# torognes/vsearch

Hardware: NVIDIA H100
Metric: usearch_global_gcups (higher is better)
Workload: dtype int16

## Files before the change

### include/vsg.h

```cpp
#ifndef VSG_H
#define VSG_H

#include <stddef.h>
#include <stdint.h>

#ifdef __cplusplus
extern "C" {
#endif

#define VSG_OK 0
#define VSG_ENODEVICE (-1)
#define VSG_ECUDA (-2)
#define VSG_EINVAL (-3)
#define VSG_ENOMEM (-4)
#define VSG_ECAP (-5)

#define VSG_SCORE_SENTINEL 32767

typedef struct vsg_ctx vsg_ctx;
typedef struct vsg_seqset vsg_seqset;
typedef struct vsg_index vsg_index;

typedef struct vsg_scoring {
  int64_t v[14];
// ... 15 lines not shown
int vsg_seqset_create(vsg_ctx * ctx, const char * cat, const int64_t * off, const int32_t * len,
                      int64_t n, int host, vsg_seqset ** out);
void vsg_seqset_destroy(vsg_seqset * s);
int64_t vsg_seqset_count(const vsg_seqset * s);
int vsg_seqset_dust(vsg_ctx * ctx, vsg_seqset * s);
int vsg_seqset_symbols(vsg_ctx * ctx, const vsg_seqset * s, uint8_t * out, int64_t cap);
int vsg_seqset_revcomp(vsg_ctx * ctx, const vsg_seqset * src, int64_t q0, int64_t n, vsg_seqset ** out);

int vsg_align_pairs(vsg_ctx * ctx, const vsg_seqset * queries, const vsg_seqset * targets,
                    int64_t npairs, const uint32_t * qidx, const uint32_t * tidx,
                    int16_t * score, uint16_t * aligned, uint16_t * matches,
                    uint16_t * mismatches, uint16_t * gaps, int32_t * trims,
                    char * cigar_buf, int64_t cigar_cap, int64_t * cigar_off);

int vsg_align_pairs_gated(vsg_ctx * ctx, const vsg_seqset * queries, const vsg_seqset * targets,
                          int64_t npairs, const uint32_t * qidx, const uint32_t * tidx,
                          int16_t * score, uint16_t * aligned, uint16_t * matches,
                          uint16_t * mismatches, uint16_t * gaps, int32_t * trims,
                          const int32_t * leader_of, double threshold, int iddef, int64_t * ck_counts);

#define VSG_STAT_SCORE 0
#define VSG_STAT_ALIGNED 1
#define VSG_STAT_MATCHES 2
#define VSG_STAT_MISMATCHES 3
#define VSG_STAT_GAPS 4
#define VSG_STAT_TRIM_LEFT 5
#define VSG_STAT_TRIM_RIGHT 6
#define VSG_STAT_CIGARLEN 7
#define VSG_STAT_WORDS 8

typedef struct vsg_profile {
  int64_t cells;
  int64_t fast_pairs;
  int64_t exact_pairs;
  int64_t fwd_launches;
  float fwd_ms;
  float traceback_ms;
  float rank_ms;
  float reserved;
  int64_t tb_skipped;
  int64_t tb_redone;
} vsg_profile;
int vsg_profile_reset(vsg_ctx * ctx);
int vsg_profile_get(vsg_ctx * ctx, vsg_profile * out);
int vsg_measure_int_peak(vsg_ctx * ctx, double * packed_lane_ops_per_s);

int vsg_index_create(vsg_ctx * ctx, const vsg_seqset * db, int wordlength, int mask_lower,
                     vsg_index ** out);
void vsg_index_destroy(vsg_index * ix);

int vsg_rank(vsg_ctx * ctx, const vsg_index * ix, const vsg_seqset * queries, int64_t q0,
             int64_t nq, int minwordmatches, int tophits, int mask_lower,
             uint32_t * cand_seqno, uint32_t * cand_count, int32_t * ncand);

typedef struct vsg_search_opts {
  double id;
  double weak_id;
  int32_t maxaccepts;
  int32_t maxrejects;
  int32_t wordlength;
  int32_t minwordmatches;
  int32_t iddef;
  int32_t strand_both;
  int32_t mask_lower;
  int32_t lazy;
  double minqt, maxqt;
  double minsl, maxsl;
  double maxid;
  double mid;
  double query_cov;
  double target_cov;
  int64_t maxsubs;
  int64_t maxgaps;
  int64_t mincols;
  int64_t maxdiffs;
  int32_t leftjust;
  int32_t rightjust;
  int64_t maxqsize;
  int64_t mintsize;
  double minsizeratio;
  double maxsizeratio;
  int32_t idprefix;
  int32_t idsuffix;
  int32_t self;
  int32_t selfid;
  int32_t qmask_dust;
  int32_t unoise;
  const int64_t * query_sizes;
  const int64_t * target_sizes;
  const int64_t * query_labels;
  const int64_t * target_labels;
  double unoise_alpha;
  int32_t sizeorder;
  int32_t reserved1;
} vsg_search_opts;

typedef struct vsg_search_result {
  int32_t target;
  int32_t matches;
  int32_t mismatches;
  int32_t gaps;
  int32_t alignment_length;
  int32_t query_length;
  int32_t target_length;
  int32_t accepted;
  int32_t strand;
// ... 324 lines not shown
```

### vsearch_b200/csrc/rank.cu

```cuda
#include "vsg_internal.h"
#include "rank_steps.cuh"

#include <cub/cub.cuh>
#include <thrust/iterator/transform_iterator.h>

#include <algorithm>
#include <cstdlib>
#include <cstring>
#include <mutex>

namespace vsg {

constexpr int CAND_CAP = 2048;
constexpr int TOPHITS_MAX = RANK_TOPHITS_MAX;
constexpr int SCAN_SEG_WORDS = 512;

template <bool FILL>
__global__ void index_build_kernel(DevSeqs db, int t0, int nt, int k, int mask_lower, int split,
                                   uint32_t * __restrict__ count ,
                                   const uint32_t * __restrict__ start, uint16_t * __restrict__ post)
{
  extern __shared__ uint32_t bitmap[];
  int const lt = blockIdx.x;
  if (lt >= nt) { return; }
  int const words = (1 << (2 * k)) >> 5;
  for (int i = threadIdx.x; i < (words > 0 ? words : 1); i += blockDim.x) { bitmap[i] = 0; }
  __syncthreads();
  int64_t const t = static_cast<int64_t>(t0) + lt;
  const uint8_t * __restrict__ s = db.sym + db.off[t];
  int const len = db.len[t];
  for (int p = k - 1 + threadIdx.x; p < len; p += blockDim.x) {
    uint32_t km;
    if (kmer_at(s, p, k, mask_lower, km)) {
      uint32_t const bit = 1u << (km & 31);
      uint32_t const old = atomicOr(&bitmap[km >> 5], bit);
      if ((old & bit) == 0) {
        uint32_t const list = split ? 2u * km + static_cast<uint32_t>(lt & 1) : km;
        if (FILL) {
          uint32_t const pos = atomicAdd(&count[list], 1u);
          post[static_cast<size_t>(start[list]) + pos] = static_cast<uint16_t>((lt & ~1) << 1);
        } else {
          atomicAdd(&count[list], 1u);
        }
      }
    }
  }
}

__global__ void pad_counts_kernel(uint32_t * __restrict__ count, int n)
{
  int const i = blockIdx.x * blockDim.x + threadIdx.x;
  if (i < n) { count[i] = (count[i] + 7u) & ~7u; }
}
__global__ void fill_u16_kernel(uint16_t * __restrict__ p, size_t n, uint16_t v)
{
  size_t const i = static_cast<size_t>(blockIdx.x) * blockDim.x + threadIdx.x;
  if (i < n) { p[i] = v; }
}

__global__ void add_totals_kernel(const uint32_t * __restrict__ count , uint32_t * __restrict__ totals, size_t hashsize)
{
  size_t const i = static_cast<size_t>(blockIdx.x) * blockDim.x + threadIdx.x;
  if (i < hashsize) { totals[i] += count[2 * i] + count[2 * i + 1]; }
}

__global__ void shard_word_counts_kernel(ShardDev S, uint32_t nlists, uint32_t * __restrict__ totals)
{
  uint32_t const i = blockIdx.x * blockDim.x + threadIdx.x;
// ... 74 lines not shown
      else { int const v2 = vr - rem * (full + 1); lane = rem + v2 / full; blk = v2 % full; }
      lp[8 * (blk * 32 + lane) + j] = x;
    }
    __syncthreads();
  }
}

template <typename T, bool DESC>
__device__ void bitonic_sort_shared(T * a, int n )
{
  for (int size = 2; size <= n; size <<= 1) {
    for (int stride = size >> 1; stride > 0; stride >>= 1) {
      __syncthreads();
      for (int i = threadIdx.x; i < (n >> 1); i += blockDim.x) {
        int const lo = 2 * i - (i & (stride - 1));
        int const hi = lo + stride;
        bool const up = ((lo & size) == 0);
        T const x = a[lo], y = a[hi];
        bool const sw = DESC ? (up ? (x < y) : (x > y)) : (up ? (x > y) : (x < y));
        if (sw) { a[lo] = y; a[hi] = x; }
      }
    }
  }
  __syncthreads();
}

__device__ __forceinline__ int next_pow2(int v)
{
  int p = 1;
  while (p < v) { p <<= 1; }
  return p;
}


__device__ __forceinline__ int threshold_from_hist(const uint32_t * hist, int top, int floor, int tophits, int & K)
{
  int const lane = threadIdx.x & 31;
  int acc = 0;
  for (; top >= floor; top -= 32) {
    int const b = top - lane;
    int const v = warp_inclusive_sum(b >= floor ? static_cast<int>(hist[b]) : 0);
    unsigned const hit = __ballot_sync(0xffffffffu, acc + v >= tophits);
    if (hit != 0u) {
      int const first = __ffs(hit) - 1;
      K = acc + __shfl_sync(0xffffffffu, v, first);
      return top - first;
    }
    acc += __shfl_sync(0xffffffffu, v, 31);
  }
  K = acc;
  return floor;
}

__device__ __forceinline__ int keep_keys_from(uint64_t * cand, int m, uint64_t tkey, int & s_ncand)
{
  uint64_t mine[CAND_CAP / RANK_THREADS];
  int cnt = 0;
  for (int i = threadIdx.x; i < m; i += blockDim.x) { uint64_t const kx = cand[i]; if (kx >= tkey) { mine[cnt++] = kx; } }
  if (threadIdx.x == 0) { s_ncand = 0; }
  __syncthreads();
  int const base = cnt > 0 ? atomicAdd(&s_ncand, cnt) : 0;
  for (int i = 0; i < cnt; i++) { cand[base + i] = mine[i]; }
  __syncthreads();
  return s_ncand;
}

__device__ __forceinline__ int sort_and_cut(uint64_t * cand, int m, int tophits)
{
  int const p2 = next_pow2(m);
  for (int i = m + threadIdx.x; i < p2; i += blockDim.x) { cand[i] = 0; }
  bitonic_sort_shared<uint64_t, true>(cand, p2);
  return m < tophits ? m : tophits;
}


__device__ __forceinline__ int query_kmers_smem(const uint8_t * __restrict__ s, int nwin, int k, int mask_lower,
                                                uint32_t * kmers, uint32_t * flag, int & s_nk, int & np2)
{
  np2 = next_pow2(nwin > 1 ? nwin : 1);
  for (int i = threadIdx.x; i < np2; i += blockDim.x) {
    uint32_t km = 0xffffffffu;
    if (i < nwin) {
      uint32_t v;
      if (kmer_at(s, i + k - 1, k, mask_lower, v)) { km = v; }
    }
    kmers[i] = km;
  }
  bitonic_sort_shared<uint32_t, false>(kmers, np2);
  int mine = 0;
  for (int i = threadIdx.x; i < np2; i += blockDim.x) {
    uint32_t const v = kmers[i];
    bool const keep = (v != 0xffffffffu) && (i == 0 || kmers[i - 1] != v);
    flag[i] = keep ? 1u : 0u;
    mine += keep;
  }
  __syncthreads();
  for (int i = threadIdx.x; i < np2; i += blockDim.x) { if (flag[i] == 0u) { kmers[i] = 0xffffffffu; } }
  atomicAdd(&s_nk, mine);
  __syncthreads();
  return s_nk;
}

__device__ __forceinline__ int query_kmers_hbm(const uint8_t * __restrict__ s, int nwin, int k, int mask_lower,
                                               uint32_t * bm, int words, uint32_t * gk, int & s_nk)
{
  if (k <= 10) {
    for (int i = threadIdx.x; i < words; i += blockDim.x) { bm[i] = 0; }
    __syncthreads();
    for (int p = threadIdx.x; p < nwin; p += blockDim.x) {
      uint32_t v;
      if (kmer_at(s, p + k - 1, k, mask_lower, v)) {
        uint32_t const bit = 1u << (v & 31);
        uint32_t const old = atomicOr(&bm[v >> 5], bit);
        if ((old & bit) == 0) { gk[atomicAdd(&s_nk, 1)] = v; }
      }
    }
  } else {
    uint32_t const hmask = static_cast<uint32_t>(words) - 1u;
    for (int i = threadIdx.x; i < words; i += blockDim.x) { bm[i] = 0xffffffffu; }
    __syncthreads();
    for (int p = threadIdx.x; p < nwin; p += blockDim.x) {
      uint32_t v;
      if (kmer_at(s, p + k - 1, k, mask_lower, v)) {
        uint32_t slot = (v * 2654435761u) >> 7 & hmask;
        for (;;) {
          uint32_t const old = atomicCAS(&bm[slot], 0xffffffffu, v);
          if (old == 0xffffffffu) { gk[atomicAdd(&s_nk, 1)] = v; break; }
          if (old == v) { break; }
          slot = (slot + 1u) & hmask;
        }
      }
    }
  }
  __threadfence_block();
  __syncthreads();
  return s_nk;
}

__device__ __forceinline__ void postings_incr(const ShardDev & S, int n, const uint32_t * lbeg, const uint32_t * llen,
                                              uint32_t * counters)
{
  int const lane = threadIdx.x & 31, warp = threadIdx.x >> 5;
  for (int li = warp; li < n; li += RANK_THREADS / 32) {
    uint32_t const len = llen[li];
    const uint32_t * __restrict__ pl = S.post32 + lbeg[li];
    for (uint32_t e = lane; e < len; e += 32) {
      uint32_t const a = __ldg(pl + e) - static_cast<uint32_t>(S.t0);
      atomicAdd(&counters[a >> 1], (a & 1) ? 0x10000u : 1u);
    }
  }
}

enum { RANK_TOP = 0, RANK_COUNT = 1, RANK_EMIT = 2 };

template <bool INCR, int MODE = RANK_TOP>
__global__ void __launch_bounds__(RANK_THREADS, 2)
rank_kernel(DevSeqs qs, int64_t q0, int nq, DevSeqs db, const ShardDev * __restrict__ shards, int nshards,
            int k, int mask_lower, int minwordmatches, int tophits,
            uint32_t * __restrict__ out_seqno, uint32_t * __restrict__ out_count, int32_t * __restrict__ out_n,
            int32_t * __restrict__ status, uint32_t * __restrict__ scratch, size_t scratch_stride, int bitmap_words,
            const int64_t * __restrict__ key_off, uint64_t * __restrict__ keys)
{
  extern __shared__ __align__(16) unsigned char smem[];
  uint64_t * const cand = reinterpret_cast<uint64_t *>(smem);
  uint32_t * const counters = reinterpret_cast<uint32_t *>(smem + CAND_CAP * 8);
  uint32_t * const kmers = counters + COUNTER_WORDS + 3;
  uint32_t * const lbeg = kmers + KMER_CAP;
  uint32_t * const llen = lbeg + KMER_CAP;
  uint32_t * const cum = llen + KMER_CAP;
  __shared__ int s_ncand, s_nk, s_T, s_K;
  __shared__ int s_wsum[RANK_THREADS / 32];

  int const lane = threadIdx.x & 31, warp = threadIdx.x >> 5;

  bool clean = false;
  for (int qi = blockIdx.x; qi < nq; qi += gridDim.x) {
    int64_t const q = q0 + qi;
    const uint8_t * __restrict__ s = qs.sym + qs.off[q];
    int const len = qs.len[q];
    int const nwin = len - k + 1;
    if (threadIdx.x == 0) { s_ncand = 0; s_nk = 0; }
    bool const longq = nwin > KMER_CAP;
    if (longq && (scratch == nullptr || nwin > 65535)) {
      if (threadIdx.x == 0) { out_n[qi] = 0; atomicExch(status, 1); }
      continue;
    }
    int np2, nk, nchunks = 1;
    uint32_t * gk = nullptr;
    if (!longq) {
      nk = query_kmers_smem(s, nwin, k, mask_lower, kmers, lbeg, s_nk, np2);
    } else {
      uint32_t * const bm = scratch + static_cast<size_t>(blockIdx.x) * scratch_stride;
      gk = bm + bitmap_words;
      nk = query_kmers_hbm(s, nwin, k, mask_lower, bm, bitmap_words, gk, s_nk);
      nchunks = nk > 0 ? (nk + KMER_CAP - 1) / KMER_CAP : 1;
      np2 = 1;
    }
    uint32_t const minmatches = static_cast<uint32_t>(minwordmatches < nk ? minwordmatches : nk);
    bool const running = MODE == RANK_TOP && !longq && (np2 + nk + 1 <= KMER_CAP);
    uint32_t * const hist = kmers + np2;
    if (running) {
      for (int i = threadIdx.x; i <= nk; i += blockDim.x) { hist[i] = 0; }
      if (threadIdx.x == 0) { s_T = static_cast<int>(minmatches); }
    }

    for (int sh = 0; sh < nshards; sh++) {
      ShardDev const S = shards[sh];
      if (!clean) { for (int i = threadIdx.x; i < COUNTER_WORDS; i += blockDim.x) { counters[i] = 0; } }
      clean = false;
      for (int chunk = 0; chunk < nchunks; chunk++) {
        if (longq) {
          int const cn = nk > 0 ? min(KMER_CAP, nk - chunk * KMER_CAP) : 1;
          for (int i = threadIdx.x; i < cn; i += blockDim.x) { kmers[i] = nk > 0 ? gk[chunk * KMER_CAP + i] : 0xffffffffu; }
          np2 = cn;
          __syncthreads();
        }
        list_bounds<INCR>(S, kmers, np2, lbeg, llen);
        __syncthreads();
        if constexpr (INCR) { postings_incr(S, np2, lbeg, llen, counters); }
        else { postings_stream(S, np2, lbeg, llen, cum, counters, s_wsum); }
        __syncthreads();
      }
      int const nwords = (S.nt + 1) >> 1;
      uint32_t thr = minmatches;
      if constexpr (MODE != RANK_TOP) {
        visit_counters<4>(counters, 0, nwords, S.nt, minmatches, true, [&](uint32_t c, int lt) {
          int const pos = atomicAdd(&s_ncand, 1);
          if (MODE == RANK_EMIT) { keys[key_off[qi] + pos] = target_key(db, S, c, lt); }
        });
        clean = true;
        __syncthreads();
        continue;
      }
      if (running) {
        uint32_t const T0 = static_cast<uint32_t>(s_T);
        visit_counters<4>(counters, 0, nwords, S.nt, T0, false, [&](uint32_t c, int) { atomicAdd(&hist[c], 1u); });
        __syncthreads();
        if (warp == 0) {
          int K;
          int const T = threshold_from_hist(hist, nk, static_cast<int>(T0), tophits, K);
          if (lane == 0) { s_T = T; s_K = K; }
        }
        int const level = s_ncand;
        __syncthreads();
        uint32_t const T1 = static_cast<uint32_t>(s_T);
        if (level + s_K <= CAND_CAP) {
          visit_counters<4>(counters, 0, nwords, S.nt, T1, true, [&](uint32_t c, int lt) {
            cand[atomicAdd(&s_ncand, 1)] = target_key(db, S, c, lt);
          });
          clean = true;
          __syncthreads();
          continue;
        }
        thr = T1;
      } else {
        int mine = 0;
        visit_counters<1>(counters, 0, nwords, S.nt, minmatches, false, [&](uint32_t, int) { mine++; });
        int total;
        int pos = block_exclusive_sum(mine, s_wsum, total);
        int const level = s_ncand;
        __syncthreads();
        if (level + total <= CAND_CAP) {
          pos += level;
          visit_counters<1>(counters, 0, nwords, S.nt, minmatches, false, [&](uint32_t c, int lt) {
            cand[pos++] = target_key(db, S, c, lt);
          });
          if (threadIdx.x == 0) { s_ncand = level + total; }
          __syncthreads();
          continue;
        }
      }
      for (int seg = 0; seg < nwords; seg += SCAN_SEG_WORDS) {
        int const level = s_ncand;
        __syncthreads();
        if (level + 2 * SCAN_SEG_WORDS > CAND_CAP) {
          int const nkeep = sort_and_cut(cand, level, tophits);
          if (threadIdx.x == 0) { s_ncand = nkeep; }
          __syncthreads();
        }
        visit_counters<1>(counters, seg, min(seg + SCAN_SEG_WORDS, nwords), S.nt, thr, false, [&](uint32_t c, int lt) {
          cand[atomicAdd(&s_ncand, 1)] = target_key(db, S, c, lt);
        });
        __syncthreads();
      }
    }
    if constexpr (MODE != RANK_TOP) {
      if (threadIdx.x == 0) { out_n[qi] = s_ncand; }
      __syncthreads();
      continue;
    }
    int m = s_ncand;
    __syncthreads();
    if (m > 2 * tophits && nk + 1 <= 2 * KMER_CAP) {
      if (!running) {
        uint32_t * const hist5 = lbeg;
        for (int i = threadIdx.x; i <= nk; i += blockDim.x) { hist5[i] = 0; }
        __syncthreads();
        for (int i = threadIdx.x; i < m; i += blockDim.x) { atomicAdd(&hist5[static_cast<uint32_t>(cand[i] >> 49)], 1u); }
        __syncthreads();
        if (warp == 0) {
          int K;
          int const T = threshold_from_hist(hist5, nk, 0, tophits, K);
          if (lane == 0) { s_T = T; }
        }
        __syncthreads();
      }
      m = keep_keys_from(cand, m, count_key(s_T), s_ncand);
    }
    int const nout = sort_and_cut(cand, m, tophits);
    for (int i = threadIdx.x; i < nout; i += blockDim.x) {
      uint64_t const key = cand[i];
      out_seqno[static_cast<size_t>(qi) * tophits + i] = 0xffffffu - static_cast<uint32_t>(key & 0xffffffu);
      out_count[static_cast<size_t>(qi) * tophits + i] = static_cast<uint32_t>(key >> 49);
    }
    if (threadIdx.x == 0) { out_n[qi] = nout; }
    __syncthreads();
  }
}

constexpr size_t RANK_SMEM = CAND_CAP * 8 + (COUNTER_WORDS + 3) * 4 + KMER_CAP * 4 * 4 + 4;

}

using namespace vsg;

struct vsg_index {
  int device = 0;
  int k = 8;
  int mask_lower = 0;
  int64_t ntargets = 0;
  const vsg_seqset * db = nullptr;
  std::vector<DevBuf> b_start, b_post, b_rkeys;
  std::vector<ShardDev> h_shards;
  DevBuf b_shards;
  int64_t total_postings = 0;
  mutable std::mutex words_lock;
  mutable DevBuf b_words;
  mutable bool words_ready = false;
};

extern "C" void vsg_index_destroy(vsg_index * ix);
namespace vsg {

static void shard_bank_order(vsg_ctx * c, const uint32_t * start, uint16_t * post, size_t nlists)
{
  if (nlists == 0) { return; }
  int sms = 132;
  cudaDeviceGetAttribute(&sms, cudaDevAttrMultiProcessorCount, c->device);
  list_bank_order_kernel<<<static_cast<int>(std::min<size_t>(nlists, static_cast<size_t>(sms) * 32)), 128, 0, c->stream>>>(start, post, static_cast<int>(nlists));
  count_launch();
}

static int build_dense_shard(vsg_ctx * c, vsg_index * ix, int sh, int t0, int nt, DevBuf & cnt, DevBuf & tmp, uint32_t * d_totals)
{
  const vsg_seqset * db = ix->db;
  int const k = ix->k;
  size_t const hashsize = static_cast<size_t>(1) << (2 * k);
  size_t const bitmap_bytes = std::max<size_t>(hashsize / 8, 4);
  size_t const nlists = 2 * hashsize;
  int rc;
  int64_t nuc = 0;
  for (int i = 0; i < nt; i++) { nuc += db->h_len[static_cast<size_t>(t0) + static_cast<size_t>(i)]; }
  if (nuc + 7 * static_cast<int64_t>(nlists) >= (static_cast<int64_t>(1) << 32) - 64) {
    Error::set("vsg_index_create: a shard of 32766 targets holds 2^32 nucleotides or more");
    return VSG_EINVAL;
  }
  DevBuf & bs = ix->b_start[static_cast<size_t>(sh)];
  if ((rc = bs.reserve(sizeof(uint32_t) * (nlists + 1))) != VSG_OK) { return rc; }
  VSG_CUDA_OK(cudaMemsetAsync(cnt.p, 0, sizeof(uint32_t) * (nlists + 1), c->stream));
  index_build_kernel<false><<<nt, 128, bitmap_bytes, c->stream>>>(db->d, t0, nt, k, ix->mask_lower, 1,
                                                                  static_cast<uint32_t *>(cnt.p), nullptr, nullptr);
  count_launch();
  if (d_totals != nullptr) {
// ... 222 lines not shown
      count_launch();
    }
    VSG_CUDA_OK(cudaStreamSynchronize(c->stream));
    VSG_CUDA_OK(cudaGetLastError());
    ix->words_ready = true;
  }
  *out = static_cast<const uint32_t *>(ix->b_words.p);
  return VSG_OK;
}
const ShardDev * index_shards(const vsg_index * ix, int & nshards)
{
  nshards = static_cast<int>(ix->h_shards.size());
  return static_cast<const ShardDev *>(ix->b_shards.p);
}

static void rank_collect_time(vsg_ctx * c)
{
  if (c->rank_pending) {
    float ms = 0.f;
    if (cudaEventElapsedTime(&ms, c->ev[4], c->ev[5]) == cudaSuccess) { c->prof_rank_ms += ms; }
    c->rank_pending = false;
  }
}

static int rank_top_alloc(vsg_ctx * c, int64_t nq, int tophits, RankTop & r)
{
  size_t const cells = static_cast<size_t>(nq) * tophits;
  int rc;
  if ((rc = c->rank_tmp.reserve(sizeof(uint32_t) * (2 * cells + nq + 4))) != VSG_OK) { return rc; }
  r.seqno = static_cast<uint32_t *>(c->rank_tmp.p);
  r.count = r.seqno + cells;
  r.n = reinterpret_cast<int32_t *>(r.count + cells);
  r.status = r.n + nq;
  VSG_CUDA_OK(cudaMemsetAsync(r.status, 0, sizeof(int32_t), c->stream));
  return VSG_OK;
}

static int rank_status(int32_t status, const char * caller)
{
  if (status == 0) { return VSG_OK; }
  Error::set(std::string(caller) + ": a query is longer than the device ranker supports (65 534 + wordlength nt)");
  return VSG_EINVAL;
}

RankTargets index_targets(const vsg_index * ix, int mask_lower)
{
  RankTargets t;
  t.shards = static_cast<const ShardDev *>(ix->b_shards.p); t.nshards = static_cast<int>(ix->h_shards.size());
  t.lens = ix->db->d; t.k = ix->k; t.mask_lower = mask_lower; t.device = ix->device;
  t.incr = false; t.timed = true;
  return t;
}

template <int MODE>
static int rank_launch(vsg_ctx * c, const RankTargets & t, const vsg_seqset * queries, int64_t q0, int64_t nq,
                       int minwordmatches, int tophits, const RankTop & out, const int64_t * d_key_off, uint64_t * d_keys)
{
  int rc;
  auto const kernel = t.incr ? rank_kernel<true, MODE> : rank_kernel<false, MODE>;
  int const k = t.k;
  VSG_CUDA_OK(cudaFuncSetAttribute(kernel, cudaFuncAttributeMaxDynamicSharedMemorySize, static_cast<int>(RANK_SMEM)));
  int sms = 132;
  cudaDeviceGetAttribute(&sms, cudaDevAttrMultiProcessorCount, c->device);
  int const grid = static_cast<int>(std::min<int64_t>(nq, static_cast<int64_t>(sms) * 2));
  int maxlen = 0;
  for (int64_t q = q0; q < q0 + nq; q++) { maxlen = std::max(maxlen, queries->h_len[static_cast<size_t>(q)]); }
  uint32_t * d_scratch = nullptr;
  size_t stride = 0;
  int bitmap_words = std::max(1, (1 << (2 * std::min(k, 10))) >> 5);
  if (k > 10) { bitmap_words = 4096; while (bitmap_words < 2 * maxlen) { bitmap_words <<= 1; } }
  if (maxlen - k + 1 > KMER_CAP) {
    stride = static_cast<size_t>(bitmap_words) + static_cast<size_t>(maxlen) + 8;
    if ((rc = c->rank_scratch.reserve(sizeof(uint32_t) * stride * static_cast<size_t>(grid))) != VSG_OK) { return rc; }
    d_scratch = static_cast<uint32_t *>(c->rank_scratch.p);
  }
  if (t.timed) { VSG_CUDA_OK(cudaEventRecord(c->ev[4], c->stream)); }
  kernel<<<grid, RANK_THREADS, RANK_SMEM, c->stream>>>(
      queries->d, q0, static_cast<int>(nq), t.lens, t.shards, t.nshards, k, t.mask_lower, minwordmatches, tophits,
      out.seqno, out.count, out.n, out.status, d_scratch, stride, bitmap_words, d_key_off, d_keys);
  count_launch();
  if (t.timed) {
    VSG_CUDA_OK(cudaEventRecord(c->ev[5], c->stream));
    c->rank_pending = true;
  }
  return VSG_OK;
}

int rank_enqueue(vsg_ctx * c, const vsg_index * ix, const vsg_seqset * queries, int64_t q0, int64_t nq,
                 int minwordmatches, int tophits, int mask_lower, RankTop & out)
{
  if (tophits < 1 || tophits > TOPHITS_MAX) { Error::set("vsg_rank: tophits must be in 1..1024"); return VSG_EINVAL; }
  if (q0 < 0 || nq < 0 || q0 + nq > queries->d.n) { Error::set("vsg_rank: query range out of bounds"); return VSG_EINVAL; }
  if (queries->device != c->device || ix->device != c->device) { Error::set("vsg_rank: sequence set / index lives on another device than the context"); return VSG_EINVAL; }
  if (nq > (1 << 30) / tophits) { Error::set("vsg_rank: batch too large"); return VSG_EINVAL; }
  int rc;
  if ((rc = rank_top_alloc(c, nq, tophits, out)) != VSG_OK || nq == 0) { return rc; }
  return rank_launch<RANK_TOP>(c, index_targets(ix, mask_lower), queries, q0, nq, minwordmatches, tophits, out, nullptr, nullptr);
}

int rank_download(vsg_ctx * c, const RankTop & r, int64_t nq, int tophits, uint32_t * h_seqno, uint32_t * h_count,
                  int32_t * h_n, const char * caller)
{
  size_t const cells = static_cast<size_t>(nq) * tophits;
  int32_t status = 0;
  if (nq > 0) {
    VSG_CUDA_OK(cudaMemcpyAsync(h_seqno, r.seqno, sizeof(uint32_t) * cells, cudaMemcpyDeviceToHost, c->stream));
    VSG_CUDA_OK(cudaMemcpyAsync(h_count, r.count, sizeof(uint32_t) * cells, cudaMemcpyDeviceToHost, c->stream));
    VSG_CUDA_OK(cudaMemcpyAsync(h_n, r.n, sizeof(int32_t) * static_cast<size_t>(nq), cudaMemcpyDeviceToHost, c->stream));
  }
  VSG_CUDA_OK(cudaMemcpyAsync(&status, r.status, sizeof(int32_t), cudaMemcpyDeviceToHost, c->stream));
  VSG_CUDA_OK(cudaStreamSynchronize(c->stream));
  rank_collect_time(c);
  return rank_status(status, caller);
}

__global__ void cut_lists_kernel(const uint64_t * __restrict__ keys, const int64_t * __restrict__ key_off,
                                 const int64_t * __restrict__ out_off, uint32_t * __restrict__ seqno, uint32_t * __restrict__ count)
{
  int const q = blockIdx.x;
  int64_t const a = key_off[q], n = out_off[q + 1] - out_off[q], o = out_off[q];
  for (int64_t i = threadIdx.x; i < n; i += blockDim.x) {
    uint64_t const key = keys[a + i];
    seqno[o + i] = 0xffffffu - static_cast<uint32_t>(key & 0xffffffu);
    count[o + i] = static_cast<uint32_t>(key >> 49);
  }
}

int rank_counts(vsg_ctx * c, const RankTargets & t, const vsg_seqset * queries, int64_t q0, int64_t nq, int minwordmatches,
                std::vector<int32_t> & n)
{
// ... 60 lines not shown
      cub::DeviceSegmentedSort::SortKeysDescending(nullptr, tb, db, static_cast<int>(keys), static_cast<int>(m), d_koff, d_koff + 1, c->stream);
      if ((rc = c->cub_tmp.reserve(tb + 64)) != VSG_OK) { return rc; }
      cub::DeviceSegmentedSort::SortKeysDescending(c->cub_tmp.p, tb, db, static_cast<int>(keys), static_cast<int>(m), d_koff, d_koff + 1, c->stream);
      count_launch();
      if (nout > 0) {
        cut_lists_kernel<<<static_cast<unsigned>(m), 256, 0, c->stream>>>(db.Current(), d_koff, d_ooff, d_seq, d_cnt);
        count_launch();
        if (t.timed) { VSG_CUDA_OK(cudaEventRecord(c->ev[5], c->stream)); }
        size_t const o = static_cast<size_t>(first[static_cast<size_t>(a)]);
        VSG_CUDA_OK(cudaMemcpyAsync(seqno.data() + o, d_seq, sizeof(uint32_t) * static_cast<size_t>(nout), cudaMemcpyDeviceToHost, c->stream));
        VSG_CUDA_OK(cudaMemcpyAsync(count.data() + o, d_cnt, sizeof(uint32_t) * static_cast<size_t>(nout), cudaMemcpyDeviceToHost, c->stream));
      }
      VSG_CUDA_OK(cudaStreamSynchronize(c->stream));
      VSG_CUDA_OK(cudaGetLastError());
      rank_collect_time(c);
    }
    a = b;
  }
  return VSG_OK;
}

}

extern "C" int vsg_rank(vsg_ctx * c, const vsg_index * ix, const vsg_seqset * queries, int64_t q0, int64_t nq,
                        int minwordmatches, int tophits, int mask_lower, uint32_t * cand_seqno,
                        uint32_t * cand_count, int32_t * ncand)
{
  if (c == nullptr || ix == nullptr || queries == nullptr || cand_seqno == nullptr || cand_count == nullptr || ncand == nullptr) {
    Error::set("vsg_rank: null argument");
    return VSG_EINVAL;
  }
  VSG_CUDA_OK(cudaSetDevice(c->device));
  if (tophits > TOPHITS_MAX) {
    std::vector<int64_t> first;
    std::vector<uint32_t> seqno, count;
    int const rc = rank_lists(c, index_targets(ix, mask_lower), queries, q0, nq, minwordmatches, tophits, first, seqno, count);
    if (rc != VSG_OK) { return rc; }
    for (int64_t i = 0; i < nq; i++) {
      size_t const a = static_cast<size_t>(first[static_cast<size_t>(i)]), n = static_cast<size_t>(first[static_cast<size_t>(i) + 1]) - a;
      std::memcpy(cand_seqno + static_cast<size_t>(i) * tophits, seqno.data() + a, sizeof(uint32_t) * n);
      std::memcpy(cand_count + static_cast<size_t>(i) * tophits, count.data() + a, sizeof(uint32_t) * n);
      ncand[i] = static_cast<int32_t>(n);
    }
    return VSG_OK;
  }
  RankTop r;
  int rc = rank_enqueue(c, ix, queries, q0, nq, minwordmatches, tophits, mask_lower, r);
  if (rc == VSG_OK) { rc = rank_download(c, r, nq, tophits, cand_seqno, cand_count, ncand, "vsg_rank"); }
  if (rc != VSG_OK) { return rc; }
  VSG_CUDA_OK(cudaGetLastError());
  return VSG_OK;
}


namespace vsg {

__global__ void cindex_append_kernel(DevSeqs db, const uint32_t * __restrict__ seqnos, int n, uint32_t first_id, int k,
                                     int mask_lower, uint32_t * __restrict__ cursor, uint32_t * __restrict__ post32,
                                     int32_t * __restrict__ clen)
{
  extern __shared__ uint32_t bitmap[];
  int const ci = blockIdx.x;
  if (ci >= n) { return; }
  int const words = (1 << (2 * k)) >> 5;
  for (int i = threadIdx.x; i < (words > 0 ? words : 1); i += blockDim.x) { bitmap[i] = 0; }
  __syncthreads();
  int64_t const t = seqnos[ci];
  const uint8_t * __restrict__ s = db.sym + db.off[t];
  int const len = db.len[t];
  if (threadIdx.x == 0) { clen[first_id + ci] = len; }
  for (int p = k - 1 + threadIdx.x; p < len; p += blockDim.x) {
    uint32_t km;
    if (kmer_at(s, p, k, mask_lower, km)) {
      uint32_t const bit = 1u << (km & 31);
      uint32_t const old = atomicOr(&bitmap[km >> 5], bit);
      if ((old & bit) == 0) { post32[atomicAdd(&cursor[km], 1u)] = first_id + static_cast<uint32_t>(ci); }
    }
  }
}

struct CIndex {
  int device = 0, k = 8, mask_lower = 0;
  const vsg_seqset * set = nullptr;
  int64_t ncent = 0;
  DevBuf b_start, b_cursor, b_post, b_clen, b_shards, b_seqnos;
  std::vector<DevBuf> b_begin;
  std::vector<uint32_t> h_seqno;
};

int cindex_create(vsg_ctx * c, const vsg_seqset * set, int wordlength, int mask_lower, CIndex ** out)
{
  *out = nullptr;
  if (wordlength < 3 || wordlength > 10) { Error::set("cluster index: the device index supports --wordlength 3..10"); return VSG_EINVAL; }
  VSG_CUDA_OK(cudaSetDevice(c->device));
  CIndex * ix = new (std::nothrow) CIndex();
  if (ix == nullptr) { Error::set("out of host memory"); return VSG_ENOMEM; }
  ix->device = c->device; ix->k = wordlength; ix->mask_lower = mask_lower; ix->set = set;
  size_t const hashsize = static_cast<size_t>(1) << (2 * wordlength);
  size_t const bitmap_bytes = std::max<size_t>(hashsize / 8, 4);
  if (bitmap_bytes > 48 * 1024) {
    VSG_CUDA_OK(cudaFuncSetAttribute(index_build_kernel<false>, cudaFuncAttributeMaxDynamicSharedMemorySize, static_cast<int>(bitmap_bytes)));
    VSG_CUDA_OK(cudaFuncSetAttribute(cindex_append_kernel, cudaFuncAttributeMaxDynamicSharedMemorySize, static_cast<int>(bitmap_bytes)));
  }
  int rc;
  DevBuf cnt, tmp;
  if ((rc = cnt.reserve(sizeof(uint32_t) * (hashsize + 1))) != VSG_OK ||
// ... 220 lines not shown
```

### vsearch_b200/csrc/rank_steps.cuh

```cuda
#pragma once

#include "vsg_internal.h"

namespace vsg {

constexpr int SHARD_BITS = 15;
constexpr int SHARD = 1 << SHARD_BITS;
constexpr int RANK_THREADS = 512;
constexpr int KMER_CAP = 2048;

constexpr int COUNTER_WORDS = SHARD / 2 + 1;
constexpr int SHARD_STATIC = SHARD - 2;
constexpr uint16_t POST_PAD = 65532;

struct ShardDev {
  const uint32_t * start;
  const uint16_t * post;
  int32_t t0;
  int32_t nt;
  const uint32_t * end;
  const uint32_t * post32;
  const uint32_t * rkeys;
  uint32_t nr;
  uint32_t reserved;
// ... 42 lines not shown
         static_cast<uint64_t>(0xffffffu - seqno);
}
__device__ __forceinline__ uint64_t target_key(const DevSeqs & db, const ShardDev & S, uint32_t count, int lt)
{
  int const t = S.t0 + lt;
  return make_key(count, static_cast<uint32_t>(db.len[t]), static_cast<uint32_t>(t));
}
__device__ __forceinline__ uint64_t count_key(int count) { return static_cast<uint64_t>(static_cast<uint32_t>(count)) << 49; }

template <typename T>
__device__ __forceinline__ T block_exclusive_sum(T x, int * s_wsum, T & total)
{
  int const lane = threadIdx.x & 31, warp = threadIdx.x >> 5;
  T const incl = warp_inclusive_sum(x);
  if (lane == 31) { s_wsum[warp] = static_cast<int>(incl); }
  __syncthreads();
  T wbase = 0;
  total = 0;
#pragma unroll
  for (int w = 0; w < RANK_THREADS / 32; w++) { T const v = static_cast<T>(s_wsum[w]); if (w < warp) { wbase += v; } total += v; }
  return wbase + incl - x;
}

template <bool INCR>
__device__ __forceinline__ void list_bounds(const ShardDev & S, const uint32_t * kmers, int n, uint32_t * lbeg, uint32_t * llen)
{
  for (int i = threadIdx.x; i < n; i += blockDim.x) {
    uint32_t const km = kmers[i];
    uint32_t b = 0, len = 0;
    if (km != 0xffffffffu) {
      if (INCR) { b = S.start[km]; len = S.end[km] - b; }
      else if (S.nr == 0u) {
        b = S.start[2 * km];
        uint32_t const mid = S.start[2 * km + 1], e = S.start[2 * km + 2];
        len = ((mid - b) >> 3) | (((e - mid) >> 3) << 16);
      } else {
        uint32_t const want = km << 1;
        uint32_t lo = 0, hi = S.nr;
        while (lo < hi) {
          uint32_t const mid = (lo + hi) >> 1;
          if (__ldg(S.rkeys + mid) < want) { lo = mid + 1; } else { hi = mid; }
        }
        b = S.start[lo];
        uint32_t na = 0, nb = 0, j = lo;
        if (j < S.nr && __ldg(S.rkeys + j) == want) { na = (S.start[j + 1] - S.start[j]) >> 3; j++; }
        if (j < S.nr && __ldg(S.rkeys + j) == (want | 1u)) { nb = (S.start[j + 1] - S.start[j]) >> 3; }
        len = na | (nb << 16);
      }
    }
    lbeg[i] = b; llen[i] = len;
  }
}

__device__ __forceinline__ void postings_stream(const ShardDev & S, int n, uint32_t * lbeg, uint32_t * llen, uint32_t * cum,
                                                uint32_t * counters, int * s_wsum)
{
  constexpr int NWARPS = RANK_THREADS / 32;
  int const lane = threadIdx.x & 31, warp = threadIdx.x >> 5;
  uint32_t Vtot;
  {
    int const per = (n + RANK_THREADS - 1) / RANK_THREADS;
    int const i0 = threadIdx.x * per;
    uint32_t nn[KMER_CAP / RANK_THREADS], bb[KMER_CAP / RANK_THREADS];
    uint32_t sum = 0;
#pragma unroll
    for (int u = 0; u < KMER_CAP / RANK_THREADS; u++) {
      bool const in = u < per && i0 + u < n;
      nn[u] = in ? llen[i0 + u] : 0u;
      bb[u] = in ? lbeg[i0 + u] : 0u;
      sum += (nn[u] & 0xffffu) + (nn[u] >> 16);
    }
    uint32_t c0 = block_exclusive_sum(sum, s_wsum, Vtot);
#pragma unroll
    for (int u = 0; u < KMER_CAP / RANK_THREADS; u++) {
      if (u < per && i0 + u < n) {
        uint32_t const na = nn[u] & 0xffffu, nv = na + (nn[u] >> 16);
        lbeg[i0 + u] = (bb[u] >> 3) - c0;
        llen[i0 + u] = c0 + na;
        cum[i0 + u] = c0 + nv;
        c0 += nv;
      }
    }
    __syncthreads();
  }
  uint32_t const per_w = ((Vtot + NWARPS * 32 - 1) / (NWARPS * 32)) * 32;
  uint32_t const wbeg = static_cast<uint32_t>(warp) * per_w;
  uint32_t const wend = min(Vtot, wbeg + per_w);
  if (wbeg < wend) {
    constexpr int U = 4;
    const uint4 * __restrict__ pbase = reinterpret_cast<const uint4 *>(S.post);
    uint32_t const cnt_sa = static_cast<uint32_t>(__cvta_generic_to_shared(counters));
    uint32_t const v_first = min(wbeg + static_cast<uint32_t>(lane), wend - 1);
    int lo = 0, hi = n - 1;
    while (lo < hi) {
      int const mid = (lo + hi) >> 1;
      if (cum[mid] <= v_first) { lo = mid + 1; } else { hi = mid; }
    }
    uint32_t sa = static_cast<uint32_t>(__cvta_generic_to_shared(lbeg + lo));
    uint32_t ce = cum[lo];
    uint4 cur[U];
    uint32_t inc[U];
    auto fetch = [&](int u, uint32_t vv) {
      inc[u] = 0u;
      if (vv < wend) {
        while (vv >= ce) {
          sa += 4u;
          asm("ld.shared.u32 %0, [%1+%2];" : "=r"(ce) : "r"(sa), "n"(2 * KMER_CAP * 4));
        }
        uint32_t vb, sp;
        asm("ld.shared.u32 %0, [%1];" : "=r"(vb) : "r"(sa));
        asm("ld.shared.u32 %0, [%1+%2];" : "=r"(sp) : "r"(sa), "n"(KMER_CAP * 4));
        cur[u] = __ldg(pbase + static_cast<uint32_t>(vb + vv));
        inc[u] = vv < sp ? 1u : 0x10000u;
      }
    };
    auto apply = [&](int u) {
      if (inc[u] != 0u) {
        uint32_t const w[4] = {cur[u].x, cur[u].y, cur[u].z, cur[u].w};
#pragma unroll
        for (int k2 = 0; k2 < 4; k2++) {
          asm volatile("red.shared.add.u32 [%0], %1;" :: "r"(cnt_sa + (w[k2] & 0xffffu)), "r"(inc[u]));
          asm volatile("red.shared.add.u32 [%0], %1;" :: "r"(cnt_sa + (w[k2] >> 16)), "r"(inc[u]));
        }
      }
    };
    for (uint32_t v0 = wbeg; v0 < wend; v0 += 32u * U) {
#pragma unroll
      for (int u = 0; u < U; u++) { fetch(u, v0 + 32u * u + static_cast<uint32_t>(lane)); }
#pragma unroll
      for (int u = 0; u < U; u++) { apply(u); }
    }
  }
}

template <int W, typename F>
__device__ __forceinline__ void visit_counters(uint32_t * counters, int w0, int w1, int nt, uint32_t thr, bool zero, F && f)
{
  static_assert(W == 1 || W == 4, "counter words per load");
  int const v1 = (w1 + W - 1) / W;
  uint32_t const below = thr > 0 ? ((thr - 1) | ((thr - 1) << 16)) : 0u;
  if (zero && threadIdx.x == 0 && nt <= SHARD_STATIC) { counters[(POST_PAD >> 2)] = 0; }
  for (int vi = w0 / W + threadIdx.x; vi < v1; vi += blockDim.x) {
    uint32_t w[W];
    if constexpr (W == 4) {
      uint4 * __restrict__ cv = reinterpret_cast<uint4 *>(counters);
      uint4 const x = cv[vi];
      if (zero) { cv[vi] = make_uint4(0u, 0u, 0u, 0u); }
      w[0] = x.x; w[1] = x.y; w[2] = x.z; w[3] = x.w;
    } else {
      w[0] = counters[vi];
      if (zero) { counters[vi] = 0u; }
    }
#pragma unroll
    for (int u = 0; u < W; u++) {
      if (W == 4 && thr > 0 && __vmaxu2(w[u], below) == below) { continue; }
      uint32_t const c0 = w[u] & 0xffffu, c1 = w[u] >> 16;
      int const lt0 = 2 * (W * vi + u), lt1 = lt0 + 1;
      if (c0 >= thr && lt0 < nt) { f(c0, lt0); }
      if (c1 >= thr && lt1 < nt) { f(c1, lt1); }
    }
  }
}

}
// ... 1 lines not shown
```

### vsearch_b200/lib.py

```python
from __future__ import annotations

import ctypes as C
import os
import re
from dataclasses import dataclass
from typing import List, Optional

import numpy as np

ROOT = os.path.dirname(os.path.dirname(os.path.abspath(__file__)))
LIB_PATH = os.environ.get("VSG_LIB") or os.path.join(ROOT, "vsearch_b200", "csrc", "libvsg.so")
HEADER = os.path.join(ROOT, "include", "vsg.h")

DEFAULT_PEN = (2, -4, 1, 1, 18, 18, 1, 1, 1, 1, 2, 2, 1, 1)
STAT_WORDS = 8

_lib = None


class VsgError(RuntimeError):
    pass


class Scoring(C.Structure):
# ... 355 lines not shown
            prof = np.zeros((0, 6), dtype=np.uint64)
            cons = np.zeros(0, dtype=np.uint8)
        _check(rc, "vsg_cluster_msa")
        return {"insertions": ins[:nins], "col_first": first, "profile": prof, "consensus": cons}

    def exact_index(self, db: SeqSetHandle) -> "ExactIndex":
        h = C.c_void_p()
        _check(load().vsg_exact_index_create(self.h, db.h, C.byref(h)), "vsg_exact_index_create")
        return ExactIndex(h)

    def search_exact(self, ix: "ExactIndex", qs: SeqSetHandle, q0: int, nq: int, opts: SearchOpts, maxhits: int = 0,
                     cap: Optional[int] = None):
        return _hits_call(lambda hits, c, first, n, _work: load().vsg_search_exact(
            self.h, ix.h, qs.h, C.c_int64(q0), C.c_int64(nq), C.byref(opts), C.c_int64(maxhits), hits, C.c_int64(c), first, n),
            nq, cap, "vsg_search_exact")

    def search_exact_command(self, query_path: str, db_path: str, /, **kw) -> dict:
        e, s, o = search_exact_opts(**kw)
        st = SearchExactStats()
        _check(load().vsg_search_exact_command(self.h, query_path.encode(), db_path.encode(), C.byref(e), C.byref(s), C.byref(o),
                                               C.byref(st)), "vsg_search_exact_command")
        return {k: getattr(st, k) for k, _ in SearchExactStats._fields_}

    def usearch_global_command(self, query_path: str, db_path: str, /, **kw) -> dict:
        u, s, o = usearch_global_opts(**kw)
        st = UsearchGlobalStats()
        _check(load().vsg_usearch_global_command(self.h, query_path.encode(), db_path.encode(), C.byref(u), C.byref(s), C.byref(o),
                                                 C.byref(st)), "vsg_usearch_global_command")
        return {k: getattr(st, k) for k, _ in UsearchGlobalStats._fields_}

    def uchime(self, input_path: str, db_path: Optional[str] = None, /, **kw) -> dict:
        o, out = uchime_opts(**kw)
        st = UchimeStats()
        _check(load().vsg_uchime_command(self.h, input_path.encode(), None if db_path is None else db_path.encode(), C.byref(o),
                                         C.byref(out), C.byref(st)), "vsg_uchime_command")
        return {k: getattr(st, k) for k, _ in UchimeStats._fields_}

    def udb_load(self, udb: "Udb"):
        sh = C.c_void_p(); ih = C.c_void_p(); ml = C.c_int(-1)
        _check(load().vsg_udb_load(self.h, udb.h, C.byref(sh), C.byref(ih), C.byref(ml)), "vsg_udb_load")
        _, _, lens = udb.sequences()
        return SeqSetHandle(self, sh, udb.n, lens), IndexHandle(ih), int(ml.value)

    def rank(self, ix: IndexHandle, qs: SeqSetHandle, q0: int, nq: int, minwordmatches: int,
             tophits: int, mask_lower: int = 0):
        seqno = np.zeros((nq, tophits), dtype=np.uint32)
        count = np.zeros((nq, tophits), dtype=np.uint32)
        nc = np.zeros(nq, dtype=np.int32)
        _check(load().vsg_rank(self.h, ix.h, qs.h, C.c_int64(q0), C.c_int64(nq), C.c_int(minwordmatches),
                               C.c_int(tophits), C.c_int(mask_lower), _ptr(seqno, C.c_uint32),
                               _ptr(count, C.c_uint32), _ptr(nc, C.c_int32)), "vsg_rank")
        return seqno, count, nc

    def sintax(self, ix: IndexHandle, qs: SeqSetHandle, q0: int, nq: int, seed: int, strand_both: int = 0,
               query_number0: Optional[int] = None, random_ties: int = 0):
        o = sintax_opts(seed, strand_both, query_number0=q0 if query_number0 is None else query_number0, random_ties=random_ties)
        res = np.zeros(nq, dtype=SINTAX_DT)
        _check(load().vsg_sintax(self.h, ix.h, qs.h, C.c_int64(q0), C.c_int64(nq), C.byref(o),
                                 res.ctypes.data_as(C.c_void_p) if nq > 0 else None), "vsg_sintax")
        return {k: res[k] for k in SINTAX_DT.names}

    def orient(self, ix: IndexHandle, qs: SeqSetHandle, q0: int, nq: int, query_mask_lower: int = 1) -> np.ndarray:
        res = np.zeros(nq, dtype=ORIENT_DT)
        _check(load().vsg_orient(self.h, ix.h, qs.h, C.c_int64(q0), C.c_int64(nq), C.c_int(query_mask_lower),
                                 res.ctypes.data_as(C.c_void_p) if nq > 0 else None), "vsg_orient")
        return np.stack([res["strand"].astype(np.int64), res["count_fwd"].astype(np.int64),
                         res["count_rev"].astype(np.int64)], axis=1)

    def search(self, ix: IndexHandle, db: SeqSetHandle, qs: SeqSetHandle, q0: int, nq: int,
               opts: SearchOpts, max_results: int):
        res = (SearchResult * (nq * max_results))()
        counts = np.zeros(nq, dtype=np.int32)
        work = np.zeros(4, dtype=np.int64)
        _check(load().vsg_search_batch(self.h, ix.h, db.h, qs.h, C.c_int64(q0), C.c_int64(nq),
                                       C.byref(opts), res, C.c_int(max_results), _ptr(counts, C.c_int32),
                                       _ptr(work, C.c_int64)), "vsg_search_batch")
        return res, counts, work

    def search_hits(self, ix: IndexHandle, db: SeqSetHandle, qs: SeqSetHandle, q0: int, nq: int,
                    opts: SearchOpts, maxhits: int = 0, cap: Optional[int] = None):
        return _hits_call(lambda hits, c, first, n, work: load().vsg_search_hits(
            self.h, ix.h, db.h, qs.h, C.c_int64(q0), C.c_int64(nq), C.byref(opts), C.c_int64(maxhits), hits, C.c_int64(c),
            first, n, work), nq, cap, "vsg_search_hits")


def _hits_call(call, nq: int, cap: Optional[int], what: str):
    first = np.zeros(nq + 1, dtype=np.int64)
    work = np.zeros(4, dtype=np.int64)
    n = C.c_int64()
    if cap is None:
        rc = call(None, 0, _ptr(first, C.c_int64), C.byref(n), _ptr(work, C.c_int64))
        if rc == 0:
            return (SearchResult * 0)(), first, work
        if rc != -5:
            _check(rc, what)
        cap = int(n.value)
    hits = (SearchResult * max(cap, 1))()
    _check(call(hits, cap, _ptr(first, C.c_int64), C.byref(n), _ptr(work, C.c_int64)), what)
    return hits, first, work


def allpairs(ctx: "Context", ss: SeqSetHandle, row0: int, nrows: int, opts: SearchOpts, cap: int):
    dt = np.dtype([("query", np.int32), ("target", np.int32), ("matches", np.int32), ("mismatches", np.int32),
                   ("gaps", np.int32), ("alignment_length", np.int32), ("nwscore", np.int32),
                   ("internal_alignment_length", np.int32), ("id", np.float64)])
    assert dt.itemsize == C.sizeof(PairHit)
# ... 545 lines not shown
```

Measured before the change: 1947.

## Add a short-query rank kernel variant with smaller shared memory for three CTAs per SM

Templates the rank kernel on a config struct and adds a short-query variant with smaller k-mer, candidate and scan-segment capacities. The variant needs about 76 KB of shared memory instead of about 115 KB, so three CTAs fit per SM instead of two. It is picked when all queries in the batch are short, tophits is at most 64 and the non-incremental path is used. The intent is more occupancy for latency-bound postings streaming. The risk is more frequent sort-and-cut passes from the smaller candidate buffer, plus register pressure at the tighter launch bound. Also adds an occupancy query API.

```diff
diff --git a/include/vsg.h b/include/vsg.h
--- a/include/vsg.h
+++ b/include/vsg.h
@@ -91,6 +91,7 @@
 int vsg_rank(vsg_ctx * ctx, const vsg_index * ix, const vsg_seqset * queries, int64_t q0,
              int64_t nq, int minwordmatches, int tophits, int mask_lower,
              uint32_t * cand_seqno, uint32_t * cand_count, int32_t * ncand);
+int vsg_rank_occupancy(vsg_ctx * ctx, int * ctas_full, int * ctas_short);
 
 typedef struct vsg_search_opts {
   double id;
diff --git a/vsearch_b200/csrc/rank.cu b/vsearch_b200/csrc/rank.cu
--- a/vsearch_b200/csrc/rank.cu
+++ b/vsearch_b200/csrc/rank.cu
@@ -11,9 +11,7 @@
 
 namespace vsg {
 
-constexpr int CAND_CAP = 2048;
 constexpr int TOPHITS_MAX = RANK_TOPHITS_MAX;
-constexpr int SCAN_SEG_WORDS = 512;
 
 template <bool FILL>
 __global__ void index_build_kernel(DevSeqs db, int t0, int nt, int k, int mask_lower, int split,
@@ -194,9 +192,10 @@
   return floor;
 }
 
+template <int CAND>
 __device__ __forceinline__ int keep_keys_from(uint64_t * cand, int m, uint64_t tkey, int & s_ncand)
 {
-  uint64_t mine[CAND_CAP / RANK_THREADS];
+  uint64_t mine[(CAND + RANK_THREADS - 1) / RANK_THREADS];
   int cnt = 0;
   for (int i = threadIdx.x; i < m; i += blockDim.x) { uint64_t const kx = cand[i]; if (kx >= tkey) { mine[cnt++] = kx; } }
   if (threadIdx.x == 0) { s_ncand = 0; }
@@ -295,8 +294,16 @@
 
 enum { RANK_TOP = 0, RANK_COUNT = 1, RANK_EMIT = 2 };
 
-template <bool INCR, int MODE = RANK_TOP>
-__global__ void __launch_bounds__(RANK_THREADS, 2)
+struct RankFull { static constexpr int CTAS = 2, KCAP = KMER_CAP, CAND = 2048, SEG = 512; };
+struct RankShort { static constexpr int CTAS = 3, KCAP = 512, CAND = 256, SEG = 64, TOPHITS = 64; };
+
+template <typename CFG>
+constexpr size_t rank_smem() { return CFG::CAND * 8 + (COUNTER_WORDS + 3) * 4 + CFG::KCAP * 4 * 4 + 4; }
+static_assert(rank_smem<RankFull>() == 114708 && rank_smem<RankShort>() == 75796, "rank_kernel's shared memory");
+static_assert(RankShort::TOPHITS + 2 * RankShort::SEG <= RankShort::CAND, "a sort-and-cut segment must fit behind tophits keys");
+
+template <typename CFG, bool INCR, int MODE = RANK_TOP>
+__global__ void __launch_bounds__(RANK_THREADS, CFG::CTAS)
 rank_kernel(DevSeqs qs, int64_t q0, int nq, DevSeqs db, const ShardDev * __restrict__ shards, int nshards,
             int k, int mask_lower, int minwordmatches, int tophits,
             uint32_t * __restrict__ out_seqno, uint32_t * __restrict__ out_count, int32_t * __restrict__ out_n,
@@ -304,12 +311,13 @@
             const int64_t * __restrict__ key_off, uint64_t * __restrict__ keys)
 {
   extern __shared__ __align__(16) unsigned char smem[];
+  constexpr int KCAP = CFG::KCAP, CAND = CFG::CAND, SEG = CFG::SEG;
   uint64_t * const cand = reinterpret_cast<uint64_t *>(smem);
-  uint32_t * const counters = reinterpret_cast<uint32_t *>(smem + CAND_CAP * 8);
+  uint32_t * const counters = reinterpret_cast<uint32_t *>(smem + CAND * 8);
   uint32_t * const kmers = counters + COUNTER_WORDS + 3;
-  uint32_t * const lbeg = kmers + KMER_CAP;
-  uint32_t * const llen = lbeg + KMER_CAP;
-  uint32_t * const cum = llen + KMER_CAP;
+  uint32_t * const lbeg = kmers + KCAP;
+  uint32_t * const llen = lbeg + KCAP;
+  uint32_t * const cum = llen + KCAP;
   __shared__ int s_ncand, s_nk, s_T, s_K;
   __shared__ int s_wsum[RANK_THREADS / 32];
 
@@ -322,7 +330,7 @@
     int const len = qs.len[q];
     int const nwin = len - k + 1;
     if (threadIdx.x == 0) { s_ncand = 0; s_nk = 0; }
-    bool const longq = nwin > KMER_CAP;
+    bool const longq = nwin > KCAP;
     if (longq && (scratch == nullptr || nwin > 65535)) {
       if (threadIdx.x == 0) { out_n[qi] = 0; atomicExch(status, 1); }
       continue;
@@ -335,11 +343,11 @@
       uint32_t * const bm = scratch + static_cast<size_t>(blockIdx.x) * scratch_stride;
       gk = bm + bitmap_words;
       nk = query_kmers_hbm(s, nwin, k, mask_lower, bm, bitmap_words, gk, s_nk);
-      nchunks = nk > 0 ? (nk + KMER_CAP - 1) / KMER_CAP : 1;
+      nchunks = nk > 0 ? (nk + KCAP - 1) / KCAP : 1;
       np2 = 1;
     }
     uint32_t const minmatches = static_cast<uint32_t>(minwordmatches < nk ? minwordmatches : nk);
-    bool const running = MODE == RANK_TOP && !longq && (np2 + nk + 1 <= KMER_CAP);
+    bool const running = MODE == RANK_TOP && !longq && (np2 + nk + 1 <= KCAP);
     uint32_t * const hist = kmers + np2;
     if (running) {
       for (int i = threadIdx.x; i <= nk; i += blockDim.x) { hist[i] = 0; }
@@ -352,15 +360,15 @@
       clean = false;
       for (int chunk = 0; chunk < nchunks; chunk++) {
         if (longq) {
-          int const cn = nk > 0 ? min(KMER_CAP, nk - chunk * KMER_CAP) : 1;
-          for (int i = threadIdx.x; i < cn; i += blockDim.x) { kmers[i] = nk > 0 ? gk[chunk * KMER_CAP + i] : 0xffffffffu; }
+          int const cn = nk > 0 ? min(KCAP, nk - chunk * KCAP) : 1;
+          for (int i = threadIdx.x; i < cn; i += blockDim.x) { kmers[i] = nk > 0 ? gk[chunk * KCAP + i] : 0xffffffffu; }
           np2 = cn;
           __syncthreads();
         }
         list_bounds<INCR>(S, kmers, np2, lbeg, llen);
         __syncthreads();
         if constexpr (INCR) { postings_incr(S, np2, lbeg, llen, counters); }
-        else { postings_stream(S, np2, lbeg, llen, cum, counters, s_wsum); }
+        else { postings_stream<KCAP>(S, np2, lbeg, llen, cum, counters, s_wsum); }
         __syncthreads();
       }
       int const nwords = (S.nt + 1) >> 1;
@@ -386,7 +394,7 @@
         int const level = s_ncand;
         __syncthreads();
         uint32_t const T1 = static_cast<uint32_t>(s_T);
-        if (level + s_K <= CAND_CAP) {
+        if (level + s_K <= CAND) {
           visit_counters<4>(counters, 0, nwords, S.nt, T1, true, [&](uint32_t c, int lt) {
             cand[atomicAdd(&s_ncand, 1)] = target_key(db, S, c, lt);
           });
@@ -402,7 +410,7 @@
         int pos = block_exclusive_sum(mine, s_wsum, total);
         int const level = s_ncand;
         __syncthreads();
-        if (level + total <= CAND_CAP) {
+        if (level + total <= CAND) {
           pos += level;
           visit_counters<1>(counters, 0, nwords, S.nt, minmatches, false, [&](uint32_t c, int lt) {
             cand[pos++] = target_key(db, S, c, lt);
@@ -412,15 +420,15 @@
           continue;
         }
       }
-      for (int seg = 0; seg < nwords; seg += SCAN_SEG_WORDS) {
+      for (int seg = 0; seg < nwords; seg += SEG) {
         int const level = s_ncand;
         __syncthreads();
-        if (level + 2 * SCAN_SEG_WORDS > CAND_CAP) {
+        if (level + 2 * SEG > CAND) {
           int const nkeep = sort_and_cut(cand, level, tophits);
           if (threadIdx.x == 0) { s_ncand = nkeep; }
           __syncthreads();
         }
-        visit_counters<1>(counters, seg, min(seg + SCAN_SEG_WORDS, nwords), S.nt, thr, false, [&](uint32_t c, int lt) {
+        visit_counters<1>(counters, seg, min(seg + SEG, nwords), S.nt, thr, false, [&](uint32_t c, int lt) {
           cand[atomicAdd(&s_ncand, 1)] = target_key(db, S, c, lt);
         });
         __syncthreads();
@@ -433,7 +441,7 @@
     }
     int m = s_ncand;
     __syncthreads();
-    if (m > 2 * tophits && nk + 1 <= 2 * KMER_CAP) {
+    if (m > 2 * tophits && nk + 1 <= 2 * KCAP) {
       if (!running) {
         uint32_t * const hist5 = lbeg;
         for (int i = threadIdx.x; i <= nk; i += blockDim.x) { hist5[i] = 0; }
@@ -447,7 +455,7 @@
         }
         __syncthreads();
       }
-      m = keep_keys_from(cand, m, count_key(s_T), s_ncand);
+      m = keep_keys_from<CAND>(cand, m, count_key(s_T), s_ncand);
     }
     int const nout = sort_and_cut(cand, m, tophits);
     for (int i = threadIdx.x; i < nout; i += blockDim.x) {
@@ -460,7 +468,6 @@
   }
 }
 
-constexpr size_t RANK_SMEM = CAND_CAP * 8 + (COUNTER_WORDS + 3) * 4 + KMER_CAP * 4 * 4 + 4;
 
 }
 
@@ -789,19 +796,30 @@
   return t;
 }
 
+static bool rank_short_fits(bool incr, int tophits, int maxlen, int k)
+{
+  int const nwin = std::max(1, maxlen - k + 1);
+  int np2 = 1;
+  while (np2 < nwin) { np2 <<= 1; }
+  return !incr && tophits <= RankShort::TOPHITS && np2 + nwin + 1 <= RankShort::KCAP;
+}
+
 template <int MODE>
 static int rank_launch(vsg_ctx * c, const RankTargets & t, const vsg_seqset * queries, int64_t q0, int64_t nq,
                        int minwordmatches, int tophits, const RankTop & out, const int64_t * d_key_off, uint64_t * d_keys)
 {
   int rc;
-  auto const kernel = t.incr ? rank_kernel<true, MODE> : rank_kernel<false, MODE>;
   int const k = t.k;
-  VSG_CUDA_OK(cudaFuncSetAttribute(kernel, cudaFuncAttributeMaxDynamicSharedMemorySize, static_cast<int>(RANK_SMEM)));
+  int maxlen = 0;
+  for (int64_t q = q0; q < q0 + nq; q++) { maxlen = std::max(maxlen, queries->h_len[static_cast<size_t>(q)]); }
+  bool const small = MODE == RANK_TOP && rank_short_fits(t.incr, tophits, maxlen, k);
+  auto const kernel = small ? rank_kernel<RankShort, false, RANK_TOP>
+                            : t.incr ? rank_kernel<RankFull, true, MODE> : rank_kernel<RankFull, false, MODE>;
+  size_t const smem = small ? rank_smem<RankShort>() : rank_smem<RankFull>();
+  VSG_CUDA_OK(cudaFuncSetAttribute(kernel, cudaFuncAttributeMaxDynamicSharedMemorySize, static_cast<int>(smem)));
   int sms = 132;
   cudaDeviceGetAttribute(&sms, cudaDevAttrMultiProcessorCount, c->device);
-  int const grid = static_cast<int>(std::min<int64_t>(nq, static_cast<int64_t>(sms) * 2));
-  int maxlen = 0;
-  for (int64_t q = q0; q < q0 + nq; q++) { maxlen = std::max(maxlen, queries->h_len[static_cast<size_t>(q)]); }
+  int const grid = static_cast<int>(std::min<int64_t>(nq, static_cast<int64_t>(sms) * (small ? RankShort::CTAS : RankFull::CTAS)));
   uint32_t * d_scratch = nullptr;
   size_t stride = 0;
   int bitmap_words = std::max(1, (1 << (2 * std::min(k, 10))) >> 5);
@@ -812,7 +830,7 @@
     d_scratch = static_cast<uint32_t *>(c->rank_scratch.p);
   }
   if (t.timed) { VSG_CUDA_OK(cudaEventRecord(c->ev[4], c->stream)); }
-  kernel<<<grid, RANK_THREADS, RANK_SMEM, c->stream>>>(
+  kernel<<<grid, RANK_THREADS, smem, c->stream>>>(
       queries->d, q0, static_cast<int>(nq), t.lens, t.shards, t.nshards, k, t.mask_lower, minwordmatches, tophits,
       out.seqno, out.count, out.n, out.status, d_scratch, stride, bitmap_words, d_key_off, d_keys);
   count_launch();
@@ -979,6 +997,19 @@
   return VSG_OK;
 }
 
+extern "C" int vsg_rank_occupancy(vsg_ctx * c, int * ctas_full, int * ctas_short)
+{
+  if (c == nullptr || ctas_full == nullptr || ctas_short == nullptr) { Error::set("vsg_rank_occupancy: null argument"); return VSG_EINVAL; }
+  VSG_CUDA_OK(cudaSetDevice(c->device));
+  auto const full = rank_kernel<RankFull, false, RANK_TOP>;
+  auto const small = rank_kernel<RankShort, false, RANK_TOP>;
+  VSG_CUDA_OK(cudaFuncSetAttribute(full, cudaFuncAttributeMaxDynamicSharedMemorySize, static_cast<int>(rank_smem<RankFull>())));
+  VSG_CUDA_OK(cudaFuncSetAttribute(small, cudaFuncAttributeMaxDynamicSharedMemorySize, static_cast<int>(rank_smem<RankShort>())));
+  VSG_CUDA_OK(cudaOccupancyMaxActiveBlocksPerMultiprocessor(ctas_full, full, RANK_THREADS, rank_smem<RankFull>()));
+  VSG_CUDA_OK(cudaOccupancyMaxActiveBlocksPerMultiprocessor(ctas_short, small, RANK_THREADS, rank_smem<RankShort>()));
+  return VSG_OK;
+}
+
 
 namespace vsg {
 
diff --git a/vsearch_b200/csrc/rank_steps.cuh b/vsearch_b200/csrc/rank_steps.cuh
--- a/vsearch_b200/csrc/rank_steps.cuh
+++ b/vsearch_b200/csrc/rank_steps.cuh
@@ -118,6 +118,7 @@
   }
 }
 
+template <int KCAP = KMER_CAP>
 __device__ __forceinline__ void postings_stream(const ShardDev & S, int n, uint32_t * lbeg, uint32_t * llen, uint32_t * cum,
                                                 uint32_t * counters, int * s_wsum)
 {
@@ -127,10 +128,10 @@
   {
     int const per = (n + RANK_THREADS - 1) / RANK_THREADS;
     int const i0 = threadIdx.x * per;
-    uint32_t nn[KMER_CAP / RANK_THREADS], bb[KMER_CAP / RANK_THREADS];
+    uint32_t nn[KCAP / RANK_THREADS], bb[KCAP / RANK_THREADS];
     uint32_t sum = 0;
 #pragma unroll
-    for (int u = 0; u < KMER_CAP / RANK_THREADS; u++) {
+    for (int u = 0; u < KCAP / RANK_THREADS; u++) {
       bool const in = u < per && i0 + u < n;
       nn[u] = in ? llen[i0 + u] : 0u;
       bb[u] = in ? lbeg[i0 + u] : 0u;
@@ -138,7 +139,7 @@
     }
     uint32_t c0 = block_exclusive_sum(sum, s_wsum, Vtot);
 #pragma unroll
-    for (int u = 0; u < KMER_CAP / RANK_THREADS; u++) {
+    for (int u = 0; u < KCAP / RANK_THREADS; u++) {
       if (u < per && i0 + u < n) {
         uint32_t const na = nn[u] & 0xffffu, nv = na + (nn[u] >> 16);
         lbeg[i0 + u] = (bb[u] >> 3) - c0;
@@ -171,11 +172,11 @@
       if (vv < wend) {
         while (vv >= ce) {
           sa += 4u;
-          asm("ld.shared.u32 %0, [%1+%2];" : "=r"(ce) : "r"(sa), "n"(2 * KMER_CAP * 4));
+          asm("ld.shared.u32 %0, [%1+%2];" : "=r"(ce) : "r"(sa), "n"(2 * KCAP * 4));
         }
         uint32_t vb, sp;
         asm("ld.shared.u32 %0, [%1];" : "=r"(vb) : "r"(sa));
-        asm("ld.shared.u32 %0, [%1+%2];" : "=r"(sp) : "r"(sa), "n"(KMER_CAP * 4));
+        asm("ld.shared.u32 %0, [%1+%2];" : "=r"(sp) : "r"(sa), "n"(KCAP * 4));
         cur[u] = __ldg(pbase + static_cast<uint32_t>(vb + vv));
         inc[u] = vv < sp ? 1u : 0x10000u;
       }
diff --git a/vsearch_b200/lib.py b/vsearch_b200/lib.py
--- a/vsearch_b200/lib.py
+++ b/vsearch_b200/lib.py
@@ -431,6 +431,11 @@
                                _ptr(count, C.c_uint32), _ptr(nc, C.c_int32)), "vsg_rank")
         return seqno, count, nc
 
+    def rank_occupancy(self):
+        full = C.c_int(); short = C.c_int()
+        _check(load().vsg_rank_occupancy(self.h, C.byref(full), C.byref(short)), "vsg_rank_occupancy")
+        return full.value, short.value
+
     def sintax(self, ix: IndexHandle, qs: SeqSetHandle, q0: int, nq: int, seed: int, strand_both: int = 0,
                query_number0: Optional[int] = None, random_ties: int = 0):
         o = sintax_opts(seed, strand_both, query_number0=q0 if query_number0 is None else query_number0, random_ties=random_ties)
```

Result: faster. 2062, median of 6 (+5.9%).
